# worldbench/lidarcrafter

Hardware: AMD Instinct MI355X
Metric: denoising-steps/sec, nuScenes 32×1024 range image, 1/2/4/8 GPU (higher is better)
Workload: dtype f16x2-split MFMA, fp32 accumulate (fp32-class accuracy)

## Files before the change

### include/lidarcrafter_hip.h

```cpp
#ifndef LIDARCRAFTER_HIP_H
#define LIDARCRAFTER_HIP_H

#include <stdint.h>

#ifdef __cplusplus
extern "C" {
#endif

#define LC_OK 0
#define LC_EINVAL (-1)
#define LC_EUNSUP (-2)

typedef void* lc_stream_t;

int lc_abi_version(void);
int lc_device_arch(char* buf, int buflen);
int lc_load_code_objects(void);

int64_t lc_packed_conv_weight_elems(int Co, int Ci, int ks);
int lc_pack_conv_weight(const float* w_oihw, float* wp, int Co, int Ci, int ks, lc_stream_t s);
int lc_conv2d_ring_fwd(const float* x, int64_t x_bs, const float* wp, const float* bias,
                       const float* res, int64_t res_bs, float* y, int64_t y_bs,
                       int B, int Ci, int Co, int H, int W, int ks, float out_scale,
                       int tile_cfg , lc_stream_t s);

int64_t lc_packed_conv_weight_f16x2_elems(int Co, int Ci, int ks);
int lc_pack_conv_weight_f16x2(const float* w_oihw, void* wp_hi, void* wp_lo, int Co, int Ci, int ks,
                              float* wmeta, lc_stream_t s);
int lc_pack_conv_weight_f16x2_dx(const float* w_fwd, void* wp_hi, void* wp_lo, int Co, int Ci, int ks,
                                 float* wmeta, const float* wmeta_fwd, lc_stream_t s);
typedef struct lc_weight_pack_job {
    const float* w;
    void *fwd_hi, *fwd_lo;
    float* fwd_meta;
    void *dx_hi, *dx_lo;
    float* dx_meta;
    int Co, Ci, ks, reserved;
} lc_weight_pack_job;
int lc_pack_conv_weights_f16x2_multi(const lc_weight_pack_job* jobs, int n, int with_dx, lc_stream_t s);
typedef struct lc_conv_range {
    float x_scale, x_unscale, amax_scaled, reserved;
} lc_conv_range;
int lc_range_from_tensor(const float* x, int64_t x_bs, int B, int64_t n, lc_conv_range* range,
                         lc_stream_t s);
int lc_range_from_amax(const float* amax, int64_t n, float bound_mult, lc_conv_range* range, lc_stream_t s);
typedef struct lc_oct_stats {
    const float* p;
    int channels, slots;
    int unit;
} lc_oct_stats;
typedef struct lc_gn_stats_input {
    const double* partials;
    int G, nch;
    float eps;
    const float *gamma, *beta, *scale, *shift;
    int64_t ss_bs;
    const lc_oct_stats *os0, *os1;
} lc_gn_stats_input;

int lc_conv2d_ring_f16x2_fwd(const float* x, int64_t x_bs, const void* wp_hi, const void* wp_lo,
                             const float* bias, const float* res, int64_t res_bs, float* y,
                             int64_t y_bs, int B, int Ci, int Co, int H, int W, int ks,
                             float out_scale, int tile_cfg ,
                             const float* gn_coeffs , int gn_cpad,
                             int gn_silu, const lc_gn_stats_input* gn_stats ,
                             float* gn_ostats_out ,
                             int gn_ostats_unit ,
                             const float* wmeta ,
                             lc_conv_range* range ,
                             lc_stream_t s);
int64_t lc_conv2d_ring_f16x2_stats_slots(int B, int Ci, int Co, int H, int W, int ks, int tile_cfg);
int64_t lc_split_act_units(int B, int C, int H, int W);
int lc_groupnorm_apply_split(const float* x, int64_t x_bs, const double* partials, const float* gamma,
                             const float* beta, const float* scale, const float* shift, int64_t ss_bs,
                             void* y_split, int B, int C, int H, int W, int G, float eps, int act_silu,
                             lc_conv_range* range, lc_stream_t s);
int lc_groupnorm_apply_os_split(const float* x, int64_t x_bs, const lc_oct_stats* s0,
                                const lc_oct_stats* s1, const float* gamma, const float* beta,
                                const float* scale, const float* shift, int64_t ss_bs, void* y_split,
                                int B, int C, int H, int W, int G, float eps, int act_silu,
                                lc_conv_range* range, lc_stream_t s);
int lc_conv2d_ring_f16x2_ps_fwd(const void* x_split, const void* wp_hi, const void* wp_lo,
                                const float* bias, const float* res, int64_t res_bs, float* y,
                                int64_t y_bs, int B, int Ci, int Co, int H, int W, float out_scale,
                                int tile_cfg, float* gn_ostats_out ,
                                int gn_ostats_unit ,
                                float* splitk_part , int ksplit,
                                const float* wmeta, lc_conv_range* range, lc_stream_t s);
int lc_conv1x1_f16x2_ps_fwd(const void* x_split, const void* wp_hi, const void* wp_lo, const float* bias,
                            const float* res, int64_t res_bs, float* y, int64_t y_bs, int B, int Ci, int Co,
                            int H, int W, float out_scale, const float* wmeta, lc_conv_range* range,
                            lc_stream_t s);
int64_t lc_splitk_stats_slots(int H, int W);
int lc_splitk_reduce(const float* part, int ksplit, const float* bias, const float* res,
                     int64_t res_bs, float* y, int64_t y_bs, int B, int Co, int H, int W,
                     float out_scale, float* gn_ostats_out, lc_stream_t s);

int lc_groupnorm_coeffs(const float* x, int64_t x_bs, const double* partials, const float* gamma,
                        const float* beta, const float* scale, const float* shift, int64_t ss_bs,
                        float* coeffs, int B, int C, int Cpad, int H, int W, int G, float eps,
                        lc_stream_t s);

int64_t lc_groupnorm_partials_elems(int B, int C, int H, int W, int G);
int lc_groupnorm_stats(const float* x, int64_t x_bs, double* partials, int B, int C, int H, int W,
                       int G, lc_stream_t s);
int lc_groupnorm_apply(const float* x, int64_t x_bs, const double* partials, const float* gamma,
                       const float* beta, const float* scale, const float* shift, int64_t ss_bs,
// ... 265 lines not shown
```

### lidarcrafter_amd/_lib.py

```python
from __future__ import annotations

import ctypes as C
import os

from .build import LIB

i32, i64, f32, f64, vp = C.c_int, C.c_int64, C.c_float, C.c_double, C.c_void_p


class CmOperand(C.Structure):
    _fields_ = [("p", vp), ("bs", i64), ("hs", i64), ("cs", i64)]


_op = C.POINTER(CmOperand)


class OctStats(C.Structure):
    _fields_ = [("p", vp), ("channels", i32), ("slots", i32), ("unit", i32)]


_os = C.POINTER(OctStats)


class GnStatsInput(C.Structure):
    _fields_ = [("partials", vp), ("G", i32), ("nch", i32), ("eps", f32), ("gamma", vp), ("beta", vp),
                ("scale", vp), ("shift", vp), ("ss_bs", i64), ("os0", _os), ("os1", _os)]


_gs = C.POINTER(GnStatsInput)


class RowSegment(C.Structure):
    _fields_ = [("p", vp), ("idx", vp), ("ld", i64), ("width", i32)]


_rs = C.POINTER(RowSegment)


class ConvRange(C.Structure):
    _fields_ = [("x_scale", f32), ("x_unscale", f32), ("amax_scaled", f32), ("reserved", f32)]


SIGNATURES = {
    "lc_abi_version": (i32, []),
    "lc_device_arch": (i32, [C.c_char_p, i32]),
    "lc_load_code_objects": (i32, []),
    "lc_packed_conv_weight_elems": (i64, [i32, i32, i32]),
    "lc_pack_conv_weight": (i32, [vp, vp, i32, i32, i32, vp]),
    "lc_conv2d_ring_fwd": (i32, [vp, i64, vp, vp, vp, i64, vp, i64, i32, i32, i32, i32, i32, i32,
                                 f32, i32, vp]),
    "lc_packed_conv_weight_f16x2_elems": (i64, [i32, i32, i32]),
    "lc_pack_conv_weight_f16x2": (i32, [vp, vp, vp, i32, i32, i32, vp, vp]),
    "lc_pack_conv_weight_f16x2_dx": (i32, [vp, vp, vp, i32, i32, i32, vp, vp, vp]),
    "lc_pack_conv_weights_f16x2_multi": (i32, [vp, i32, i32, vp]),
    "lc_range_from_amax": (i32, [vp, i64, f32, vp, vp]),
    "lc_groupnorm_amax_partials": (i64, [i32, i32, i32, i32, i32, i32]),
    "lc_conv2d_ring_f16x2_fwd": (i32, [vp, i64, vp, vp, vp, vp, i64, vp, i64, i32, i32, i32, i32,
                                       i32, i32, f32, i32, vp, i32, i32, _gs, vp, i32, vp, vp, vp]),
    "lc_split_act_units": (i64, [i32, i32, i32, i32]),
    "lc_groupnorm_apply_split": (i32, [vp, i64, vp, vp, vp, vp, vp, i64, vp, i32, i32, i32, i32, i32,
                                       f32, i32, vp, vp]),
    "lc_groupnorm_apply_os_split": (i32, [vp, i64, _os, _os, vp, vp, vp, vp, i64, vp, i32, i32, i32,
                                          i32, i32, f32, i32, vp, vp]),
    "lc_conv1x1_f16x2_ps_fwd": (i32, [vp, vp, vp, vp, vp, i64, vp, i64, i32, i32, i32, i32, i32, f32, vp, vp, vp]),
    "lc_conv2d_ring_f16x2_ps_fwd": (i32, [vp, vp, vp, vp, vp, i64, vp, i64, i32, i32, i32, i32, i32,
                                          f32, i32, vp, i32, vp, i32, vp, vp, vp]),
    "lc_range_from_tensor": (i32, [vp, i64, i32, i64, vp, vp]),
    "lc_splitk_stats_slots": (i64, [i32, i32]),
    "lc_splitk_reduce": (i32, [vp, i32, vp, vp, i64, vp, i64, i32, i32, i32, i32, f32, vp, vp]),
    "lc_conv2d_ring_f16x2_stats_slots": (i64, [i32, i32, i32, i32, i32, i32, i32]),
    "lc_groupnorm_coeffs": (i32, [vp, i64, vp, vp, vp, vp, vp, i64, vp, i32, i32, i32, i32, i32,
                                  i32, f32, vp]),
    "lc_groupnorm_partials_elems": (i64, [i32, i32, i32, i32, i32]),
    "lc_groupnorm_stats": (i32, [vp, i64, vp, i32, i32, i32, i32, i32, vp]),
    "lc_groupnorm_apply": (i32, [vp, i64, vp, vp, vp, vp, vp, i64, vp, i64, i32, i32, i32, i32,
                                 i32, f32, i32, vp]),
    "lc_groupnorm_apply_train": (i32, [vp, i64, vp, vp, vp, vp, vp, i64, vp, i64, i32, i32, i32, i32,
                                       i32, f32, i32, vp, vp, vp]),
    "lc_groupnorm_apply_os": (i32, [vp, i64, _os, _os, vp, vp, vp, vp, i64, vp, i64, i32, i32, i32,
                                    i32, i32, f32, i32, vp]),
    "lc_conv2d_ring_wgrad_scratch_elems": (i64, [i32, i32, i32, i32, i32, i32]),
    "lc_conv2d_ring_wgrad": (i32, [vp, i64, vp, i64, vp, vp, vp, i32, i32, i32, i32, i32, i32, i32, vp]),
    "lc_conv2d_ring_wgrad_f16x2": (i32, [vp, i64, vp, i64, vp, vp, vp, vp, vp, i32, i32, i32, i32, i32,
                                         i32, i32, vp]),
    "lc_groupnorm_meanrstd": (i32, [vp, i64, vp, vp, i32, i32, i32, i32, i32, f32, vp]),
    "lc_groupnorm_bwd": (i32, [vp, i64, vp, i64, vp, vp, vp, vp, vp, i64, vp, vp, i64, i32, i32, i32,
                               i32, i32, i32, vp]),
    "lc_groupnorm_bwd_train": (i32, [vp, i64, vp, i64, vp, vp, vp, vp, vp, i64, vp, vp, i64, vp, vp, vp, vp,
                                     i32, i32, i32, i32, i32, i32, vp, vp]),
    "lc_resample2x_fwd": (i32, [vp, i64, vp, i64, i32, i32, i32, i32, i32, vp]),
    "lc_resample2x_stats_slots": (i64, [i32, i32, i32]),
    "lc_resample2x_stats_fwd": (i32, [vp, i64, vp, i64, i32, i32, i32, i32, i32, vp, vp]),
    "lc_linear_fwd": (i32, [vp, vp, vp, vp, i32, i32, i32, i32, i32, vp]),
    "lc_sinusoid_fwd": (i32, [vp, vp, i32, i32, f32, vp]),
    "lc_attention_fwd": (i32, [_op, _op, _op, _op, _op, _op, _op, _op, vp, i64, i64, i64,
                               i32, i32, i32, i32, i32, i32, i32, i32, f32, vp]),
    "lc_attention_f16x2_fwd": (i32, [_op, _op, _op, _op, _op, _op, _op, _op, vp, i64, i64, i64,
                                     i32, i32, i32, i32, i32, i32, i32, i32, f32, vp]),
    "lc_conv1x1_f16x2_ps_qkv_fwd": (i32, [vp, vp, vp, vp, vp, i64, vp, i32, i32, i32, i32, i32, i32, vp, vp, vp]),
    "lc_groupnorm_coeffs_os": (i32, [_os, _os, vp, vp, vp, vp, i64, vp, i32, i32, i32, i32, f32, vp]),
    "lc_resample2x_pair_fwd": (i32, [vp, i64, vp, i32, vp, i64, vp, i64, i32, i32, i32, i32, i32, vp]),
    "lc_split_act_fwd": (i32, [vp, i64, vp, i32, i32, i32, i32, vp, vp]),
    "lc_up2_combine9_stats_slots": (i64, [i32, i32]),
    "lc_up2_combine9_fwd": (i32, [vp, i64, vp, vp, i64, i32, i32, i32, i32, vp, vp]),
    "lc_up2_combine9_xup_fwd": (i32, [vp, i64, vp, vp, i64, vp, i64, vp, i64, i32, i32, i32, i32, vp, vp]),
    "lc_attention_units_elems": (i64, [i32, i32, i32, i32]),
    "lc_attention_pack_units": (i32, [_op, vp, i32, i32, i32, i32, i32, i32, i32, i32, i32, vp]),
    "lc_attention_units_fwd": (i32, [_op, _op, vp, vp, i64, i64, i64, i32, i32, i32, i32, i32, i32, i32, i32, f32, vp]),
    "lc_qk_norm_cm_fwd": (i32, [vp, i64, i64, vp, i64, i64, vp, vp, i32, i32, i32, i32, vp]),
    "lc_flow_step_fwd": (i32, [vp, i64, vp, i64, vp, vp, i64, i32, i64, vp]),
    "lc_hdit_rmsnorm_fwd": (i32, [vp, i64, i64, vp, i64, i32, vp, i64, i64, i32, i32, i32, f32, vp]),
    "lc_hdit_geglu_fwd": (i32, [vp, i64, vp, i64, i32, i32, i32, vp]),
    "lc_hdit_qk_prep_fwd": (i32, [vp, i64, i64, vp, i64, i64, vp, vp, vp, i32, i32, i32, i32, vp]),
    "lc_hdit_na_fwd": (i32, [_op, _op, _op, vp, i64, i64, i64, i32, i32, i32, i32, i32, i32, i32, f32, vp]),
    "lc_hdit_space_to_depth_fwd": (i32, [vp, i64, vp, i64, i32, i32, i32, i32, i32, i32, vp]),
    "lc_hdit_depth_to_space_fwd": (i32, [vp, i64, vp, i64, vp, i64, vp, i32, i32, i32, i32, i32, i32, vp]),
    "lc_hdit_tokenize_fwd": (i32, [vp, i64, vp, vp, vp, i64, i32, i32, i32, i32, i32, i32, vp]),
    "lc_hdit_fourier_fwd": (i32, [vp, vp, vp, i32, i32, vp]),
    "lc_hdit_na_train_fwd": (i32, [_op, _op, _op, vp, i64, i64, i64, vp, i32, i32, i32, i32, i32, i32, i32, f32, vp]),
    "lc_hdit_rmsnorm_bwd": (i32, [vp, i64, i64, vp, i64, i32, vp, i64, i64, vp, i64, i64, vp, vp, i64, i32, i32, i32,
                                  f32, vp]),
    "lc_hdit_geglu_bwd": (i32, [vp, i64, vp, i64, vp, i64, i32, i32, i32, vp]),
    "lc_hdit_qk_prep_bwd": (i32, [vp, i64, i64, vp, i64, i64, vp, i64, i64, vp, i64, i64, vp, i64, i64, vp, i64, i64,
                                  vp, vp, vp, vp, vp, i32, i32, i32, i32, vp]),
    "lc_hdit_na_bwd": (i32, [_op, _op, _op, _op, _op, vp, vp, vp, vp, vp, i32, i32, i32, i32, i32, i32, i32, f32, vp]),
    "lc_hdit_lerp_bwd": (i32, [vp, i64, vp, i64, vp, i64, vp, vp, i64, vp, i64, vp, i32, i32, i32, i32, i32, i32, vp]),
    "lc_groupnorm_jvp_partials_elems": (i64, [i32, i32, i32, i32, i32]),
    "lc_groupnorm_jvp_stats": (i32, [vp, i64, vp, i64, vp, i32, i32, i32, i32, i32, vp]),
    "lc_groupnorm_jvp_apply_train": (i32, [vp, i64, vp, i64, vp, vp, vp, vp, vp, vp, vp, i64, vp, i64, vp, i64,
                                           i32, i32, i32, i32, i32, f32, i32, vp, vp, vp, vp]),
    "lc_qk_norm_cm_jvp": (i32, [vp, i64, i64, vp, i64, i64, vp, vp, i64, i64, vp, i64, i64, i32, i32, i32, i32, vp]),
    "lc_qk_norm_cm_bwd_partials": (i64, [i32, i32, i32]),
    "lc_qk_norm_cm_bwd": (i32, [vp, i64, i64, vp, i64, i64, vp, vp, i64, i64, vp, vp, i32, i32, i32, i32, vp]),
# ... 102 lines not shown
```

### lidarcrafter_amd/build.py

```python
from __future__ import annotations

import os
import shutil
import subprocess
import sys

HERE = os.path.dirname(os.path.abspath(__file__))
CSRC = os.path.join(HERE, "csrc")
LIB = os.path.join(HERE, "liblidarcrafter_hip.so")
LIB_P1 = os.path.join(HERE, "liblidarcrafter_hip_p1.so")
SOURCES = ["conv.hip", "conv_f16x2.hip", "conv_f16x2_tall.hip", "conv_f16x2_s2.hip", "norm.hip", "resample.hip", "upfold.hip", "misc.hip", "attention.hip", "attention_units.hip", "geometry.hip", "roipool.hip", "lidar.hip", "layout.hip", "temporal.hip", "metrics.hip", "voxel.hip", "conv_bwd.hip", "attention_bwd.hip", "attention_bwd_h.hip", "flow.hip", "flow_jvp.hip", "hdit.hip", "hdit_bwd.hip", "layout_gen.hip"]


def hipcc() -> str:
    for cand in (os.environ.get("HIPCC"), shutil.which("hipcc"), "/opt/rocm/bin/hipcc"):
        if cand and os.path.exists(cand):
            return cand
    raise RuntimeError("hipcc not found (need ROCm); cannot build the HIP hot path")


def needs_build() -> bool:
    if not os.path.exists(LIB):
        return True
    if not os.path.exists(LIB_P1):
        return True
    t = min(os.path.getmtime(LIB), os.path.getmtime(LIB_P1))
    deps = [os.path.join(CSRC, f) for f in os.listdir(CSRC)]
    deps.append(os.path.join(os.path.dirname(HERE), "include", "lidarcrafter_hip.h"))
    return any(os.path.getmtime(d) > t for d in deps)


def build(force: bool = False, verbose: bool = True) -> str:
    if not force and not needs_build():
        return LIB
    objs = []
    os.makedirs(os.path.join(HERE, "build"), exist_ok=True)
    procs = []
    for src in SOURCES:
        obj = os.path.join(HERE, "build", src.replace(".hip", ".o"))
        cmd = [hipcc(), "--offload-arch=gfx950", "-O3", "-std=c++17", "-fPIC", "-Wno-inline-asm", "-c",
               os.path.join(CSRC, src), "-o", obj] + os.environ.get("LC_EXTRA_HIPCC_FLAGS", "").split()
        procs.append((cmd, subprocess.Popen(cmd, stdout=subprocess.PIPE, stderr=subprocess.STDOUT)))
        objs.append(obj)
    p1_objs = []
    for src in ("conv_f16x2.hip", "conv_f16x2_tall.hip"):
        p1_obj = os.path.join(HERE, "build", src.replace(".hip", "_p1.o"))
        cmd = [hipcc(), "--offload-arch=gfx950", "-O3", "-std=c++17", "-fPIC", "-Wno-inline-asm", "-DLC_F16X2_TERMS=1", "-c",
               os.path.join(CSRC, src), "-o", p1_obj] + os.environ.get("LC_EXTRA_HIPCC_FLAGS", "").split()
        procs.append((cmd, subprocess.Popen(cmd, stdout=subprocess.PIPE, stderr=subprocess.STDOUT)))
        p1_objs.append(p1_obj)
    for cmd, p in procs:
        out, _ = p.communicate()
        if p.returncode != 0:
            raise RuntimeError("hipcc failed: %s\n%s" % (" ".join(cmd), out.decode()))
        if verbose and out.strip():
            print(out.decode())
    cmd = [hipcc(), "--offload-arch=gfx950", "-shared", "-fPIC", "-o", LIB] + objs
    subprocess.run(cmd, check=True)
    subprocess.run([hipcc(), "--offload-arch=gfx950", "-shared", "-fPIC", "-o", LIB_P1] + p1_objs, check=True)
    if verbose:
        print("built", LIB, "and", os.path.basename(LIB_P1))
    return LIB


if __name__ == "__main__":
    build(force="--force" in sys.argv)
```

### lidarcrafter_amd/csrc/misc.hip

```cpp
#include "common.h"

namespace {

template <int MT>
__global__ __launch_bounds__(256) void linear_kernel(const float* __restrict__ x,
                                                    const float* __restrict__ w,
                                                    const float* __restrict__ b,
                                                    float* __restrict__ y, int M, int K, int N,
                                                    int act_in, int act_out) {
    const int lane = threadIdx.x & 63;
    const int n = blockIdx.x * 4 + (threadIdx.x >> 6);
    const int m0 = blockIdx.y * MT;
    if (n >= N) return;
    float acc[MT];
#pragma unroll
    for (int i = 0; i < MT; ++i) acc[i] = 0.f;
    const float* wr = w + (long long)n * K;
    for (int k = lane; k < K; k += 64) {
        const float wv = wr[k];
#pragma unroll
        for (int i = 0; i < MT; ++i) {
            if (m0 + i < M) {
                float xv = x[(long long)(m0 + i) * K + k];
                if (act_in) xv = lc_silu(xv);
// ... 99 lines not shown
                                                  long long n) {
    const int b = blockIdx.y;
    const float* xp = x + b * x_bs;
    float* yp = y + b * y_bs;
    for (long long i = blockIdx.x * 256ll + threadIdx.x; i < n; i += (long long)gridDim.x * 256)
        yp[i] = xp[i];
}

__global__ __launch_bounds__(256) void add_scale_kernel(const float* __restrict__ a, long long a_bs,
                                                       const float* __restrict__ bb, long long b_bs,
                                                       float* __restrict__ y, long long y_bs,
                                                       long long n, float scale) {
    const int b = blockIdx.y;
    const float* ap = a + b * a_bs;
    const float* bp = bb + b * b_bs;
    float* yp = y + b * y_bs;
    for (long long i = blockIdx.x * 256ll + threadIdx.x; i < n; i += (long long)gridDim.x * 256)
        yp[i] = (ap[i] + bp[i]) * scale;
}

typedef _Float16 cal_half8 __attribute__((ext_vector_type(8)));
__global__ __launch_bounds__(512) void calib_mfma_kernel(const cal_half8* __restrict__ ops, int iters, float* __restrict__ sink) {
    f32x16 acc[4];
#pragma unroll
    for (int i = 0; i < 4; ++i)
#pragma unroll
        for (int r = 0; r < 16; ++r) acc[i][r] = 0.f;
    const int t = blockIdx.x * 512 + threadIdx.x;
    cal_half8 a[2], b[2];
    a[0] = ops[4 * t]; a[1] = ops[4 * t + 1]; b[0] = ops[4 * t + 2]; b[1] = ops[4 * t + 3];
    for (int it = 0; it < iters; ++it) {
#pragma unroll
        for (int rep = 0; rep < 4; ++rep)
#pragma unroll
            for (int i = 0; i < 4; ++i)
                acc[i] = __builtin_amdgcn_mfma_f32_32x32x16_f16(a[i & 1], b[(i >> 1) ^ (rep & 1)], acc[i], 0, 0, 0);
    }
    float s = 0.f;
#pragma unroll
    for (int i = 0; i < 4; ++i)
#pragma unroll
        for (int r = 0; r < 16; ++r) s += acc[i][r];
    sink[t] = s;
}
__global__ __launch_bounds__(256) void calib_copy_kernel(const f32x4* __restrict__ src, f32x4* __restrict__ dst, long long n4) {
    for (long long i = blockIdx.x * 256ll + threadIdx.x; i < n4; i += (long long)gridDim.x * 256)
        dst[i] = __builtin_nontemporal_load(src + i);
}

inline int grid_for(long long n) {
    long long g = (n + 255) / 256;
    return (int)(g > 4096 ? 4096 : (g < 1 ? 1 : g));
}

}

extern "C" int lc_abi_version(void) { return 5; }

extern "C" int64_t lc_calibrate_mfma_f16(const void* operands, int blocks, int iters, float* sink, lc_stream_t s) {
    if (!operands || !sink || blocks <= 0 || iters <= 0) return LC_EINVAL;
    hipLaunchKernelGGL(calib_mfma_kernel, dim3(blocks), dim3(512), 0, lc_s(s), reinterpret_cast<const cal_half8*>(operands),
                       iters, sink);
    const int rc = lc_launch_status();
    if (rc != LC_OK) return rc < 0 ? rc : -rc;
    return 2ll * 32 * 32 * 16 * 16 * (int64_t)iters * 8 * blocks;
}

extern "C" int lc_calibrate_stream_copy(const float* src, float* dst, int64_t n, lc_stream_t s) {
    if (!src || !dst || n <= 0 || (n & 3) || ((uintptr_t)src & 15) || ((uintptr_t)dst & 15)) return LC_EINVAL;
    hipLaunchKernelGGL(calib_copy_kernel, dim3(8192), dim3(256), 0, lc_s(s), reinterpret_cast<const f32x4*>(src),
                       reinterpret_cast<f32x4*>(dst), (long long)(n / 4));
    return lc_launch_status();
}

extern "C" {
int lc_touch_attention();
int lc_touch_attention_bwd();
int lc_touch_attention_bwd_h();
int lc_touch_conv();
int lc_touch_conv_bwd();
int lc_touch_conv_f16x2();
int lc_touch_conv_f16x2_tall();
int lc_touch_conv_f16x2_s2();
int lc_touch_geometry();
int lc_touch_layout();
int lc_touch_lidar();
int lc_touch_metrics();
int lc_touch_norm();
int lc_touch_resample();
int lc_touch_roipool();
int lc_touch_temporal();
int lc_touch_upfold();
int lc_touch_voxel();
}
extern "C" int lc_load_code_objects(void) {
    int (*const touch[])() = {lc_touch_attention, lc_touch_attention_bwd, lc_touch_attention_bwd_h, lc_touch_conv, lc_touch_conv_bwd, lc_touch_conv_f16x2, lc_touch_conv_f16x2_tall, lc_touch_conv_f16x2_s2, lc_touch_geometry, lc_touch_layout, lc_touch_lidar, lc_touch_metrics, lc_touch_norm, lc_touch_resample, lc_touch_roipool, lc_touch_temporal, lc_touch_upfold, lc_touch_voxel};
    for (auto f : touch) {
        const int rc = f();
        if (rc != 0) return rc;
    }
    hipFuncAttributes fa;
    return (int)hipFuncGetAttributes(&fa, reinterpret_cast<const void*>(&linear_kernel<8>));
}

extern "C" int lc_device_arch(char* buf, int buflen) {
    if (!buf || buflen <= 0) return LC_EINVAL;
    int dev = 0;
    hipError_t e = hipGetDevice(&dev);
    if (e != hipSuccess) return (int)e;
    hipDeviceProp_t p;
    e = hipGetDeviceProperties(&p, dev);
    if (e != hipSuccess) return (int)e;
    int i = 0;
    for (; i < buflen - 1 && p.gcnArchName[i]; ++i) buf[i] = p.gcnArchName[i];
    buf[i] = 0;
    return LC_OK;
}

extern "C" int lc_linear_fwd(const float* x, const float* w, const float* b, float* y, int M, int K,
                             int N, int act_in, int act_out, lc_stream_t s) {
    if (!x || !w || !y || M <= 0 || K <= 0 || N <= 0) return LC_EINVAL;
    constexpr int MT = 8;
    dim3 grid((N + 3) / 4, (M + MT - 1) / MT);
    hipLaunchKernelGGL(linear_kernel<MT>, grid, dim3(256), 0, lc_s(s), x, w, b, y, M, K, N, act_in,
                       act_out);
    return lc_launch_status();
}

extern "C" int lc_sinusoid_fwd(const float* t, float* y, int M, int channels, float max_period,
                               lc_stream_t s) {
    if (!t || !y || M <= 0 || channels < 4 || (channels & 1)) return LC_EINVAL;
    const int n = M * (channels / 2);
    hipLaunchKernelGGL(sinusoid_kernel, dim3((n + 255) / 256), dim3(256), 0, lc_s(s), t, y, M,
                       channels, max_period);
    return lc_launch_status();
}

extern "C" int lc_pstep_fwd(const float* x_t, int64_t xt_bs, const float* pred, int64_t pred_bs,
                            const float* noise, int64_t noise_bs, const float* coef, float* x_s,
                            int64_t xs_bs, int B, int64_t n, int objective, int mode,
                            lc_stream_t s) {
    if (!x_t || !pred || !coef || !x_s || B <= 0 || n <= 0) return LC_EINVAL;
    if (objective < 0 || objective > 2 || mode < 0 || mode > 3) return LC_EINVAL;
    hipLaunchKernelGGL(pstep_kernel, dim3(grid_for(n), B), dim3(256), 0, lc_s(s), x_t,
                       (long long)xt_bs, pred, (long long)pred_bs, noise, (long long)noise_bs, coef,
                       x_s, (long long)xs_bs, (long long)n, objective, mode);
    return lc_launch_status();
}

extern "C" int lc_copy_strided(const float* x, int64_t x_bs, float* y, int64_t y_bs, int B,
                               int64_t n, lc_stream_t s) {
    if (!x || !y || B <= 0 || n <= 0) return LC_EINVAL;
    hipLaunchKernelGGL(copy_kernel, dim3(grid_for(n), B), dim3(256), 0, lc_s(s), x, (long long)x_bs,
                       y, (long long)y_bs, (long long)n);
    return lc_launch_status();
}

extern "C" int lc_add_scale(const float* a, int64_t a_bs, const float* b, int64_t b_bs, float* y,
                            int64_t y_bs, int B, int64_t n, float scale, lc_stream_t s) {
    if (!a || !b || !y || B <= 0 || n <= 0) return LC_EINVAL;
    hipLaunchKernelGGL(add_scale_kernel, dim3(grid_for(n), B), dim3(256), 0, lc_s(s), a,
                       (long long)a_bs, b, (long long)b_bs, y, (long long)y_bs, (long long)n, scale);
    return lc_launch_status();
}

extern "C" int lc_gate_bias_act(const float* x, int64_t x_bs, const float* gate_logit,
                                const float* bias, int64_t gb_bs, const float* res, int64_t res_bs,
                                float* y, int64_t y_bs, int B, int C, int N, int act, lc_stream_t s) {
    if (!x || !gate_logit || !bias || !y || B <= 0 || C <= 0 || N <= 0 || act < 0 || act > 1)
        return LC_EINVAL;
    hipLaunchKernelGGL(gate_bias_kernel, dim3(C, B), dim3(256), 0, lc_s(s), x, (long long)x_bs,
                       gate_logit, bias, (long long)gb_bs, res, (long long)res_bs, y,
                       (long long)y_bs, C, N, act);
    return lc_launch_status();
}
```

### lidarcrafter_amd/ops.py

```python
from __future__ import annotations

from typing import Optional

import torch

from ._lib import check, lib

_F32 = torch.float32
_HALF = (torch.float16, torch.bfloat16)


def _stream() -> int:
    return torch.cuda.current_stream().cuda_stream


def _req(t: torch.Tensor, name: str) -> None:
    if not isinstance(t, torch.Tensor) or not t.is_cuda:
        raise RuntimeError(f"lidarcrafter_amd.ops: `{name}` must be a CUDA(HIP) tensor -- the hot "
                           "path has no CPU fallback (oracle/ holds the CPU restatement for tests)")
    if t.dtype != _F32:
        raise TypeError(f"`{name}` must be float32, got {t.dtype} (float16 / bfloat16 INPUTS are "
                        "up-cast at the op boundary, e.g. under torch.autocast; `out=` tensors and "
                        "other dtypes are not)")

# ... 678 lines not shown
            check(lib().lc_pack_conv_weights_f16x2_multi(self.table.data_ptr(), len(self.order), 1, _stream()),
                  "lc_pack_conv_weights_f16x2_multi")
        for e in self.order:
            base = e["base"]()
            Co, Ci, ks, _ = e["shape"]
            ver = base._version
            e["packed_version"] = ver
            f, b = e["fwd"], e["bwd"]
            f.Co, f.Ci, f.ks, f._key = Co, Ci, ks, (e["ptr"], ver, e["shape"])
            f._w4, f.wp, f.wh, f.wl, f.wmeta = base.detach().view(e["shape"]), None, e["fh"], e["fl"], e["fmeta"]
            b.Co, b.Ci, b.ks, b._key = Ci, Co, ks, ("dx", e["ptr"], ver, e["shape"])
            b._w4, b.wp, b.wh, b.wl, b.wmeta = f._w4, None, e["dh"], e["dl"], e["dmeta"]
        return len(self.order)


_train_weight_plans = {}


def train_weight_plan(device) -> TrainWeightPlan:
    plan = _train_weight_plans.get(device)
    if plan is None:
        plan = _train_weight_plans[device] = TrainWeightPlan(device)
    return plan


def prepare_model(module: torch.nn.Module) -> int:
    n = 0
    dev = None
    for m in module.modules():
        d = m.__dict__
        pairs = []
        if isinstance(d.get("_packed"), PackedConv) and isinstance(getattr(m, "weight", None), torch.Tensor):
            pairs.append((d["_packed"], m.weight))
        if isinstance(d.get("_pk_in"), PackedConv):
            att = getattr(m, "attn", None)
            if att is not None and getattr(att, "in_proj_weight", None) is not None:
                pairs.append((d["_pk_in"], att.in_proj_weight[:, :, None, None]))
                pairs.append((d["_pk_out"], att.out_proj.weight[:, :, None, None]))
            elif att is not None and getattr(att, "qkv", None) is not None:
                pairs.append((d["_pk_in"], att.qkv.weight[:, :, None, None]))
                pairs.append((d["_pk_out"], att.proj.weight[:, :, None, None]))
        for pk, w in pairs:
            if not w.is_cuda or w.dim() not in (3, 4) or w.shape[-1] not in (1, 3):
                continue
            dev = w.device
            with torch.cuda.device(dev):
                if CONV_PRECISION == "f16x2":
                    pk.get_f16x2(w)
                else:
                    pk.get(w)
            n += 1
    if dev is not None:
        with torch.cuda.device(dev):
            rc = int(lib().lc_load_code_objects())
        if rc != 0:
            import warnings

            warnings.warn(f"lc_load_code_objects: hipError {rc} while pre-loading the kernels' code objects; continuing "
                          "(they load at their first launch)")
    return n


def range_from_amax(amax: torch.Tensor, packed: PackedConv, device, bound_mult: float = 1.0) -> None:
    ptr = packed.range_ptr(device)
    packed._arena.device_managed.add(packed._slot)
    check(lib().lc_range_from_amax(amax.data_ptr(), amax.numel(), float(bound_mult), ptr, _stream()),
          "lc_range_from_amax")


def range_from_tensor(x: torch.Tensor, packed: PackedConv) -> None:
    _req(x, "x")
    B = x.shape[0]
    n = x.numel() // B
    if x.dim() == 4:
        x_bs = _bs4(x, "x")
    else:
        x = x if x.is_contiguous() else x.contiguous()
        x_bs = n
    ptr = packed.range_ptr(x.device)
    packed._arena.device_managed.add(packed._slot)
    check(lib().lc_range_from_tensor(x.data_ptr(), x_bs, B, n, ptr, _stream()), "lc_range_from_tensor")


def conv2d_ring(x: torch.Tensor, packed: PackedConv, weight: torch.Tensor,
                bias: Optional[torch.Tensor] = None, res: Optional[torch.Tensor] = None,
                out: Optional[torch.Tensor] = None, out_scale: float = 1.0,
                tile_cfg: int = 0, precision: Optional[str] = None,
                gn_coeffs: Optional[torch.Tensor] = None, gn_silu: bool = True,
                emit_stats: bool = False, dx_of: Optional[PackedConv] = None,
                weight_is_fwd: bool = False) -> torch.Tensor:
    if isinstance(x, SplitAct):
        return _conv2d_ring_presplit(x, packed, weight, bias, res, out, out_scale, tile_cfg,
                                     emit_stats)
    x_bs = _bs4(x, "x")
    prec = precision or CONV_PRECISION
    if gn_coeffs is not None and prec != "f16x2":
        raise ValueError("fused input GroupNorm exists for the f16x2 conv kernels only")
    if weight_is_fwd and prec != "f16x2":
        raise ValueError("weight_is_fwd exists for the f16x2 kernels only")
    if prec == "f16x2":
        wh, wl = packed.get_f16x2_dx(weight, dx_of) if weight_is_fwd else packed.get_f16x2(weight)
    else:
        wp = packed.get(weight)
    B, Ci, H, W = x.shape
    if Ci != packed.Ci:
        raise ValueError(f"conv: input has {Ci} channels, weight expects {packed.Ci}")
    Co = packed.Co
    if out is None:
        out = torch.empty((B, Co, H, W), device=x.device, dtype=_F32)
    y_bs = _bs4(out, "out")
    if tuple(out.shape) != (B, Co, H, W):
        raise ValueError(f"conv: out shape {tuple(out.shape)} != {(B, Co, H, W)}")
    r_bs = 0
    if res is not None:
        r_bs = _bs4(res, "res")
        if tuple(res.shape) != (B, Co, H, W):
            raise ValueError("conv: residual shape mismatch")
    if bias is not None:
        _req(bias, "bias")
    ks = packed.ks
    _drop_stats(out)
    with _Timed("conv3x3" if ks == 3 else "conv1x1", 2.0 * B * H * W * Co * Ci * ks * ks,
                rd=4.0 * (B * Ci * H * W + Co * Ci * ks * ks + (B * Co * H * W if res is not None else 0)),
                wr=4.0 * B * Co * H * W):
        if prec == "f16x2":
            cpad = 0
            gs_ref = None
            if isinstance(gn_coeffs, GnStats):
                if gn_coeffs.shape != (B, Ci, H, W):
                    raise ValueError("conv: GroupNorm statistics belong to a different tensor")
                gs_ref, gn_coeffs = gn_coeffs.byref(), None
            if gn_coeffs is not None:
                _req(gn_coeffs, "gn_coeffs")
                if gn_coeffs.dim() != 3 or gn_coeffs.shape[0] != B or gn_coeffs.shape[2] != 4 or \
                        not gn_coeffs.is_contiguous():
                    raise ValueError("gn_coeffs must be contiguous [B, Cpad, 4]")
                cpad = gn_coeffs.shape[1]
            sbuf, slots = None, 0
            unit = 2 if (emit_stats is not True and int(emit_stats) in (2, 4)) else 8
            if emit_stats and PRODUCER_GN_STATS and (unit == 8 or ks == 3):
                slots = int(lib().lc_conv2d_ring_f16x2_stats_slots(B, Ci, Co, H, W, ks, int(tile_cfg)))
                if slots > 0:
                    sbuf = torch.empty((B, Co // unit, slots, 4), device=x.device, dtype=_F32)
            check(_conv_lib().lc_conv2d_ring_f16x2_fwd(x.data_ptr(), x_bs, wh.data_ptr(), wl.data_ptr(),
                                                 _p(bias), _p(res), r_bs, out.data_ptr(), y_bs, B,
                                                 Ci, Co, H, W, ks, float(out_scale),
                                                 int(tile_cfg), _p(gn_coeffs), cpad, int(gn_silu),
                                                 gs_ref, _p(sbuf), unit, packed.wmeta.data_ptr(),
                                                 packed.range_ptr(x.device), _stream()),
                  "lc_conv2d_ring_f16x2_fwd")
            if sbuf is not None:
                _attach_stats(out, _OctStatsHandle(sbuf, Co, slots, (B, H * W), unit))
        else:
            check(lib().lc_conv2d_ring_fwd(x.data_ptr(), x_bs, wp.data_ptr(), _p(bias), _p(res),
                                           r_bs, out.data_ptr(), y_bs, B, Ci, Co, H, W, ks,
                                           float(out_scale), int(tile_cfg), _stream()),
                  "lc_conv2d_ring_fwd")
    return out


def _conv2d_ring_presplit(xs: SplitAct, packed: PackedConv, weight, bias, res, out, out_scale,
                          tile_cfg, emit_stats) -> torch.Tensor:
    if xs.packed is not packed:
        raise ValueError("conv: the pre-split activation was produced for another layer "
                         "(its x_scale belongs to that layer's range record)")
    wh, wl = packed.get_f16x2(weight)
    B, Ci, H, W = xs.shape
    if Ci != packed.Ci or packed.ks not in (1, 3):
        raise ValueError("conv: pre-split input needs a 1x1 / 3x3 kernel with matching channels")
    Co = packed.Co
    dev = xs.buf.device
    if out is None:
        out = torch.empty((B, Co, H, W), device=dev, dtype=_F32)
    y_bs = _bs4(out, "out")
    if tuple(out.shape) != (B, Co, H, W):
        raise ValueError(f"conv: out shape {tuple(out.shape)} != {(B, Co, H, W)}")
    r_bs = 0
    if res is not None:
        r_bs = _bs4(res, "res")
        if tuple(res.shape) != (B, Co, H, W):
            raise ValueError("conv: residual shape mismatch")
    if bias is not None:
# ... 1443 lines not shown
```

Baseline: 272.0.

## Add FP32 direct 3x3 conv kernel for thin output-channel convs

Adds a dedicated FP32 FMA kernel for 3x3 circular-padded convolutions with at most 4 output channels, such as the final output projection. It stages input tiles in LDS with register prefetch and keeps all weights in shared memory. Input channels are split across the four waves, and partial sums are reduced through LDS. This avoids the f16x2 MFMA path, whose tiles would be mostly padding for tiny Co, at the cost of scalar FMA throughput and an extra code path to maintain.

```diff
diff --git a/include/lidarcrafter_hip.h b/include/lidarcrafter_hip.h
--- a/include/lidarcrafter_hip.h
+++ b/include/lidarcrafter_hip.h
@@ -23,6 +23,10 @@
                        const float* res, int64_t res_bs, float* y, int64_t y_bs,
                        int B, int Ci, int Co, int H, int W, int ks, float out_scale,
                        int tile_cfg , lc_stream_t s);
+
+int lc_conv2d_ring_thin_co_fwd(const float* x, int64_t x_bs, const float* w_oihw, const float* bias,
+                               const float* res, int64_t res_bs, float* y, int64_t y_bs,
+                               int B, int Ci, int Co, int H, int W, float out_scale, lc_stream_t s);
 
 int64_t lc_packed_conv_weight_f16x2_elems(int Co, int Ci, int ks);
 int lc_pack_conv_weight_f16x2(const float* w_oihw, void* wp_hi, void* wp_lo, int Co, int Ci, int ks,
diff --git a/lidarcrafter_amd/_lib.py b/lidarcrafter_amd/_lib.py
--- a/lidarcrafter_amd/_lib.py
+++ b/lidarcrafter_amd/_lib.py
@@ -49,6 +49,7 @@
     "lc_pack_conv_weight": (i32, [vp, vp, i32, i32, i32, vp]),
     "lc_conv2d_ring_fwd": (i32, [vp, i64, vp, vp, vp, i64, vp, i64, i32, i32, i32, i32, i32, i32,
                                  f32, i32, vp]),
+    "lc_conv2d_ring_thin_co_fwd": (i32, [vp, i64, vp, vp, vp, i64, vp, i64, i32, i32, i32, i32, i32, f32, vp]),
     "lc_packed_conv_weight_f16x2_elems": (i64, [i32, i32, i32]),
     "lc_pack_conv_weight_f16x2": (i32, [vp, vp, vp, i32, i32, i32, vp, vp]),
     "lc_pack_conv_weight_f16x2_dx": (i32, [vp, vp, vp, i32, i32, i32, vp, vp, vp]),
diff --git a/lidarcrafter_amd/build.py b/lidarcrafter_amd/build.py
--- a/lidarcrafter_amd/build.py
+++ b/lidarcrafter_amd/build.py
@@ -9,7 +9,7 @@
 CSRC = os.path.join(HERE, "csrc")
 LIB = os.path.join(HERE, "liblidarcrafter_hip.so")
 LIB_P1 = os.path.join(HERE, "liblidarcrafter_hip_p1.so")
-SOURCES = ["conv.hip", "conv_f16x2.hip", "conv_f16x2_tall.hip", "conv_f16x2_s2.hip", "norm.hip", "resample.hip", "upfold.hip", "misc.hip", "attention.hip", "attention_units.hip", "geometry.hip", "roipool.hip", "lidar.hip", "layout.hip", "temporal.hip", "metrics.hip", "voxel.hip", "conv_bwd.hip", "attention_bwd.hip", "attention_bwd_h.hip", "flow.hip", "flow_jvp.hip", "hdit.hip", "hdit_bwd.hip", "layout_gen.hip"]
+SOURCES = ["conv.hip", "conv_f16x2.hip", "conv_f16x2_tall.hip", "conv_f16x2_s2.hip", "conv_thin_co.hip", "norm.hip", "resample.hip", "upfold.hip", "misc.hip", "attention.hip", "attention_units.hip", "geometry.hip", "roipool.hip", "lidar.hip", "layout.hip", "temporal.hip", "metrics.hip", "voxel.hip", "conv_bwd.hip", "attention_bwd.hip", "attention_bwd_h.hip", "flow.hip", "flow_jvp.hip", "hdit.hip", "hdit_bwd.hip", "layout_gen.hip"]
 
 
 def hipcc() -> str:
diff --git a/lidarcrafter_amd/csrc/conv_thin_co.hip b/lidarcrafter_amd/csrc/conv_thin_co.hip
--- /dev/null
+++ b/lidarcrafter_amd/csrc/conv_thin_co.hip
@@ -0,0 +1,219 @@
+#include "common.h"
+
+namespace {
+
+constexpr int TH = 8, TW = 64, CK = 16, CW = CK / 4, ROWS = TH + 2, PITCH = TW + 8, GROUPS = PITCH / 4;
+constexpr int STAGE_F4 = CK * ROWS * GROUPS;
+constexpr int NLD = (STAGE_F4 + 255) / 256;
+constexpr int STAGE_FLOATS = CK * ROWS * PITCH;
+constexpr int MAX_W_FLOATS = 4608;
+
+struct ThinArgs {
+    const float* x; const float* w; const float* bias; const float* res; float* y;
+    long long x_bs, res_bs, y_bs;
+    int Ci, Co, H, W, tiles_h, tiles_w, vec_io;
+    float out_scale;
+};
+
+template <int CO> struct VecOf;
+template <> struct VecOf<1> { typedef float T; };
+template <> struct VecOf<2> { typedef float T __attribute__((ext_vector_type(2))); };
+template <> struct VecOf<4> { typedef float T __attribute__((ext_vector_type(4))); };
+
+template <int CO> __device__ __forceinline__ float lane_of(const typename VecOf<CO>::T& v, int i) { return v[i]; }
+template <> __device__ __forceinline__ float lane_of<1>(const float& v, int) { return v; }
+
+template <int CO>
+__global__ __launch_bounds__(256) void conv_thin_co_kernel(ThinArgs a) {
+    typedef typename VecOf<CO>::T vec;
+    constexpr int RED_FLOATS = 3 * 8 * CO * 64;
+    constexpr int XS_FLOATS = STAGE_FLOATS > RED_FLOATS ? STAGE_FLOATS : RED_FLOATS;
+    __shared__ __attribute__((aligned(16))) float xs[XS_FLOATS];
+    __shared__ __attribute__((aligned(16))) float ws[MAX_W_FLOATS];
+
+    const int tid = threadIdx.x, lane = tid & 63, wave = tid >> 6;
+    int t = blockIdx.x;
+    const int tw_i = t % a.tiles_w; t /= a.tiles_w;
+    const int th_i = t % a.tiles_h;
+    const int b = t / a.tiles_h;
+    const int h0 = th_i * TH, c0 = tw_i * TW;
+    const int H = a.H, W = a.W, Wg = W >> 2;
+    const long long plane = (long long)H * W;
+    const float* xb = a.x + b * a.x_bs;
+
+    const int Cip = (a.Ci + CK - 1) / CK * CK;
+    for (int e = tid; e < Cip * 9 * CO; e += 256) {
+        const int co = e % CO, r = e / CO;
+        ws[e] = (co < a.Co && r < a.Ci * 9) ? a.w[(long long)co * a.Ci * 9 + r] : 0.0f;
+    }
+
+    int g_off[NLD];
+    unsigned live = 0, inside = 0;
+#pragma unroll
+    for (int k = 0; k < NLD; ++k) {
+        const int idx = tid + k * 256;
+        const int ck = idx / (ROWS * GROUPS), rem = idx % (ROWS * GROUPS);
+        const int row = rem / GROUPS, g = rem % GROUPS;
+        const int gh = h0 - 1 + row;
+        int gg = (c0 >> 2) - 1 + g;
+        gg %= Wg;
+        if (gg < 0) gg += Wg;
+        g_off[k] = 0;
+        if (idx < STAGE_F4) {
+            live |= 1u << k;
+            if (gh >= 0 && gh < H) {
+                inside |= 1u << k;
+                g_off[k] = (int)(ck * plane + (long long)gh * W + gg * 4);
+            }
+        }
+    }
+
+    f32x4 pre[NLD];
+    auto fetch = [&](int ci0) {
+        const float* xc = xb + ci0 * plane;
+#pragma unroll
+        for (int k = 0; k < NLD; ++k) {
+            pre[k] = f32x4{0.0f, 0.0f, 0.0f, 0.0f};
+            if ((inside & (1u << k)) && ci0 + (tid + k * 256) / (ROWS * GROUPS) < a.Ci)
+                pre[k] = *reinterpret_cast<const f32x4*>(xc + g_off[k]);
+        }
+    };
+    auto put = [&]() {
+#pragma unroll
+        for (int k = 0; k < NLD; ++k)
+            if (live & (1u << k)) *reinterpret_cast<f32x4*>(&xs[(tid + k * 256) * 4]) = pre[k];
+    };
+
+    const int r = lane >> 3, cg = lane & 7;
+    vec acc[8];
+#pragma unroll
+    for (int p = 0; p < 8; ++p) acc[p] = vec(0.0f);
+
+    fetch(0);
+    put();
+    __syncthreads();
+    for (int ci0 = 0; ci0 < a.Ci; ci0 += CK) {
+        const bool more = ci0 + CK < a.Ci;
+        if (more) fetch(ci0 + CK);
+#pragma unroll
+        for (int cc = 0; cc < CW; ++cc) {
+            const int ck = wave * CW + cc;
+            const float* xr = &xs[(ck * ROWS + r) * PITCH + cg * 8 + 3];
+            const vec* wr = reinterpret_cast<const vec*>(ws) + (ci0 + ck) * 9;
+#pragma unroll
+            for (int dy = 0; dy < 3; ++dy) {
+                float v[10];
+                const float* p0 = xr + dy * PITCH;
+                v[0] = p0[0];
+                const f32x4 m0 = *reinterpret_cast<const f32x4*>(p0 + 1);
+                const f32x4 m1 = *reinterpret_cast<const f32x4*>(p0 + 5);
+                v[9] = p0[9];
+#pragma unroll
+                for (int i = 0; i < 4; ++i) { v[1 + i] = m0[i]; v[5 + i] = m1[i]; }
+#pragma unroll
+                for (int dx = 0; dx < 3; ++dx) {
+                    const vec wv = wr[dy * 3 + dx];
+#pragma unroll
+                    for (int p = 0; p < 8; ++p) {
+                        if constexpr (CO == 1) acc[p] = fmaf(v[p + dx], wv, acc[p]);
+                        else acc[p] = __builtin_elementwise_fma(vec(v[p + dx]), wv, acc[p]);
+                    }
+                }
+            }
+        }
+        __syncthreads();
+        if (more) {
+            put();
+            __syncthreads();
+        }
+    }
+
+    if (wave > 0) {
+#pragma unroll
+        for (int p = 0; p < 8; ++p)
+#pragma unroll
+            for (int co = 0; co < CO; ++co)
+                xs[((wave - 1) * 8 * CO + p * CO + co) * 64 + lane] = lane_of<CO>(acc[p], co);
+    }
+    __syncthreads();
+    if (wave > 0) return;
+
+    const int h = h0 + r, c = c0 + cg * 8;
+    if (h >= H) return;
+    const bool q0 = c < W, q1 = c + 4 < W;
+    if (!q0) return;
+#pragma unroll
+    for (int co = 0; co < CO; ++co) {
+        if (co >= a.Co) break;
+        float o[8];
+#pragma unroll
+        for (int p = 0; p < 8; ++p) {
+            float s = lane_of<CO>(acc[p], co);
+#pragma unroll
+            for (int w2 = 0; w2 < 3; ++w2) s += xs[(w2 * 8 * CO + p * CO + co) * 64 + lane];
+            o[p] = s;
+        }
+        const float bv = a.bias ? a.bias[co] : 0.0f;
+        const long long off = (long long)co * plane + (long long)h * W + c;
+        float* yp = a.y + b * a.y_bs + off;
+        const float* rp = a.res ? a.res + b * a.res_bs + off : nullptr;
+        if (a.vec_io) {
+#pragma unroll
+            for (int q = 0; q < 2; ++q) {
+                if (q == 1 && !q1) break;
+                f32x4 rv = f32x4{0.0f, 0.0f, 0.0f, 0.0f};
+                if (rp) rv = *reinterpret_cast<const f32x4*>(rp + 4 * q);
+                f32x4 out;
+#pragma unroll
+                for (int i = 0; i < 4; ++i) {
+                    float s = o[4 * q + i] + bv;
+                    if (rp) s += rv[i];
+                    out[i] = s * a.out_scale;
+                }
+                *reinterpret_cast<f32x4*>(yp + 4 * q) = out;
+            }
+        } else {
+#pragma unroll
+            for (int p = 0; p < 8; ++p) {
+                if (p >= 4 && !q1) break;
+                float s = o[p] + bv;
+                if (rp) s += rp[p];
+                yp[p] = s * a.out_scale;
+            }
+        }
+    }
+}
+
+template <int CO>
+int launch_thin(const ThinArgs& a, int B, hipStream_t st) {
+    hipLaunchKernelGGL(conv_thin_co_kernel<CO>, dim3(B * a.tiles_h * a.tiles_w), dim3(256), 0, st, a);
+    return lc_launch_status();
+}
+
+}
+
+extern "C" int lc_conv2d_ring_thin_co_fwd(const float* x, int64_t x_bs, const float* w_oihw, const float* bias,
+                                          const float* res, int64_t res_bs, float* y, int64_t y_bs, int B, int Ci,
+                                          int Co, int H, int W, float out_scale, lc_stream_t s) {
+    if (!x || !w_oihw || !y || B <= 0 || Ci <= 0 || Co <= 0 || H <= 0 || W <= 0) return LC_EINVAL;
+    const int cop = Co == 3 ? 4 : Co;
+    if (Co > 4 || Ci % 8 != 0 || W % 4 != 0 || cop * ((Ci + CK - 1) / CK * CK) * 9 > MAX_W_FLOATS) return LC_EUNSUP;
+    if ((long long)CK * H * W >= (1LL << 31)) return LC_EUNSUP;
+    if ((reinterpret_cast<uintptr_t>(x) & 15) || (x_bs & 3)) return LC_EUNSUP;
+    ThinArgs a;
+    a.x = x; a.w = w_oihw; a.bias = bias; a.res = res; a.y = y;
+    a.x_bs = x_bs; a.res_bs = res_bs; a.y_bs = y_bs;
+    a.Ci = Ci; a.Co = Co; a.H = H; a.W = W;
+    a.tiles_h = (H + TH - 1) / TH; a.tiles_w = (W + TW - 1) / TW;
+    a.vec_io = !(reinterpret_cast<uintptr_t>(y) & 15) && !(y_bs & 3) &&
+               (!res || (!(reinterpret_cast<uintptr_t>(res) & 15) && !(res_bs & 3)));
+    a.out_scale = out_scale;
+    if ((long long)B * a.tiles_h * a.tiles_w >= (1LL << 31)) return LC_EUNSUP;
+    switch (cop) {
+        case 1: return launch_thin<1>(a, B, lc_s(s));
+        case 2: return launch_thin<2>(a, B, lc_s(s));
+        default: return launch_thin<4>(a, B, lc_s(s));
+    }
+}
+
+LC_TOUCH_TU(conv_thin_co, conv_thin_co_kernel<2>)
diff --git a/lidarcrafter_amd/csrc/misc.hip b/lidarcrafter_amd/csrc/misc.hip
--- a/lidarcrafter_amd/csrc/misc.hip
+++ b/lidarcrafter_amd/csrc/misc.hip
@@ -205,6 +205,7 @@
 int lc_touch_conv_f16x2();
 int lc_touch_conv_f16x2_tall();
 int lc_touch_conv_f16x2_s2();
+int lc_touch_conv_thin_co();
 int lc_touch_geometry();
 int lc_touch_layout();
 int lc_touch_lidar();
@@ -217,7 +218,7 @@
 int lc_touch_voxel();
 }
 extern "C" int lc_load_code_objects(void) {
-    int (*const touch[])() = {lc_touch_attention, lc_touch_attention_bwd, lc_touch_attention_bwd_h, lc_touch_conv, lc_touch_conv_bwd, lc_touch_conv_f16x2, lc_touch_conv_f16x2_tall, lc_touch_conv_f16x2_s2, lc_touch_geometry, lc_touch_layout, lc_touch_lidar, lc_touch_metrics, lc_touch_norm, lc_touch_resample, lc_touch_roipool, lc_touch_temporal, lc_touch_upfold, lc_touch_voxel};
+    int (*const touch[])() = {lc_touch_attention, lc_touch_attention_bwd, lc_touch_attention_bwd_h, lc_touch_conv, lc_touch_conv_bwd, lc_touch_conv_f16x2, lc_touch_conv_f16x2_tall, lc_touch_conv_f16x2_s2, lc_touch_conv_thin_co, lc_touch_geometry, lc_touch_layout, lc_touch_lidar, lc_touch_metrics, lc_touch_norm, lc_touch_resample, lc_touch_roipool, lc_touch_temporal, lc_touch_upfold, lc_touch_voxel};
     for (auto f : touch) {
         const int rc = f();
         if (rc != 0) return rc;
diff --git a/lidarcrafter_amd/ops.py b/lidarcrafter_amd/ops.py
--- a/lidarcrafter_amd/ops.py
+++ b/lidarcrafter_amd/ops.py
@@ -784,6 +784,39 @@
     check(lib().lc_range_from_tensor(x.data_ptr(), x_bs, B, n, ptr, _stream()), "lc_range_from_tensor")
 
 
+THIN_CO = _os.environ.get("LC_THIN_CO", "1") != "0"
+
+
+def thin_co_conv(Ci: int, Co: int, ks: int, W: int) -> bool:
+    return THIN_CO and ks == 3 and Co <= 4 and Ci % 8 == 0 and W % 4 == 0 and \
+        (4 if Co == 3 else Co) * ((Ci + 15) // 16 * 16) <= 512
+
+
+def _conv2d_ring_thin_co(x, x_bs, packed: PackedConv, bias, res, out, out_scale) -> torch.Tensor:
+    B, Ci, H, W = x.shape
+    Co = packed.Co
+    if out is None:
+        out = torch.empty((B, Co, H, W), device=x.device, dtype=_F32)
+    y_bs = _bs4(out, "out")
+    if tuple(out.shape) != (B, Co, H, W):
+        raise ValueError(f"conv: out shape {tuple(out.shape)} != {(B, Co, H, W)}")
+    r_bs = 0
+    if res is not None:
+        r_bs = _bs4(res, "res")
+        if tuple(res.shape) != (B, Co, H, W):
+            raise ValueError("conv: residual shape mismatch")
+    if bias is not None:
+        _req(bias, "bias")
+    _drop_stats(out)
+    with _Timed("conv3x3", 2.0 * B * H * W * Co * Ci * 9,
+                rd=4.0 * (B * Ci * H * W + Co * Ci * 9 + (B * Co * H * W if res is not None else 0)),
+                wr=4.0 * B * Co * H * W):
+        check(lib().lc_conv2d_ring_thin_co_fwd(x.data_ptr(), x_bs, packed._w4.data_ptr(), _p(bias), _p(res), r_bs,
+                                               out.data_ptr(), y_bs, B, Ci, Co, H, W, float(out_scale), _stream()),
+              "lc_conv2d_ring_thin_co_fwd")
+    return out
+
+
 def conv2d_ring(x: torch.Tensor, packed: PackedConv, weight: torch.Tensor,
                 bias: Optional[torch.Tensor] = None, res: Optional[torch.Tensor] = None,
                 out: Optional[torch.Tensor] = None, out_scale: float = 1.0,
@@ -800,6 +833,14 @@
         raise ValueError("fused input GroupNorm exists for the f16x2 conv kernels only")
     if weight_is_fwd and prec != "f16x2":
         raise ValueError("weight_is_fwd exists for the f16x2 kernels only")
+    if precision is None and prec == "f16x2" and THIN_CO and tile_cfg == 0 and gn_coeffs is None and not weight_is_fwd and \
+            weight.dim() == 4 and weight.shape[0] <= 4 and conv_products() == 3 and \
+            thin_co_conv(weight.shape[1], weight.shape[0], weight.shape[2], x.shape[3]) and \
+            x.data_ptr() % 16 == 0 and x_bs % 4 == 0:
+        packed._refresh(weight)
+        if x.shape[1] != packed.Ci:
+            raise ValueError(f"conv: input has {x.shape[1]} channels, weight expects {packed.Ci}")
+        return _conv2d_ring_thin_co(x, x_bs, packed, bias, res, out, out_scale)
     if prec == "f16x2":
         wh, wl = packed.get_f16x2_dx(weight, dx_of) if weight_is_fwd else packed.get_f16x2(weight)
     else:
```

After: 272.6 (median of 6 runs). Within noise of the previous version (+0.2%).
